# cbalint13/opencv-dlco

Hardware: AMD Instinct MI355X
Metric: pj-learn patch-pairs/sec (higher is better)
Workload: dtype f32; 1 GPU; pj-learn configs[1] Liberty-shaped, rank ~64: 500000 pair-rows x PR-dim 8192, batch 200+200 per GPU (global 200+200), mu=0.0025 gamma=0.5, fp32, rank 48 after 3893 steps; device= (gfx950:sramecc+:xnack-), burn_in_steps=300

## Files before the change

include/dlco.h:

```cpp
#ifndef DLCO_H
#define DLCO_H

#include <stddef.h>
#include <stdint.h>

#ifdef __cplusplus
extern "C" {
#endif

#define DLCO_OK            0
#define DLCO_ERR_INVALID  -2
#define DLCO_ERR_HIP      -3
#define DLCO_ERR_NODEVICE -4
#define DLCO_ERR_NOCONV   -5
#define DLCO_ERR_COMM     -6

typedef struct dlco_ctx dlco_ctx;

typedef struct dlco_cfg {
    int32_t  F;
    int32_t  N;
    int32_t  B;
    float    mu;
    float    gamma;
// ... 95 lines not shown
    int32_t split_k, k_dev, small_m_tiles, small_n_tiles, depth, reps;
    float   alpha, beta, b1, b2;
    const float *E1_host, *E2_host;
} dlco_gemm_probe_args;
int dlco_gemm_probe(dlco_ctx *ctx, const dlco_gemm_probe_args *args, float *C_host, float *C2_host, int32_t *depth_used,
                    double *us_per_launch);
int dlco_chol_probe(dlco_ctx *ctx, const float *M_host, int32_t n, int32_t ld, float rel_thresh, float *Linv_host,
                    int32_t *dead_host);
typedef struct dlco_ortho_probe_args {
    const float *Z_host, *Zprev_host, *Gp_host;
    int32_t m, panel_end, n_lock, unfused;
    float   alpha, b1, b2;
} dlco_ortho_probe_args;
int dlco_ortho_probe(dlco_ctx *ctx, const dlco_ortho_probe_args *args, float *Qo_host, float *Yb_host, float *T_host,
                     int64_t fused[2]);
int dlco_fused_counters(const dlco_ctx *ctx, int64_t out[2]);
int dlco_hinge_sum(dlco_ctx *ctx, const float *pos_host, int32_t n_pos,
                   const float *neg_host, int32_t n_neg, double *out);
int dlco_roc_stats(dlco_ctx *ctx, const float *dist_host, const uint8_t *labels_host, int32_t n,
                   float *fpr95, double *auc);

typedef struct dlco_log_entry {
    uint32_t t;
    int32_t  is_best;
    int32_t  saved;
    float    loss_val, regul, obj, obj_best;
    int32_t  rank, rank_best;
    int32_t  dim;
    double   auc, auc_best;
    float    fpr95, fpr95_best;
// ... 234 lines not shown
```

opencv-dlco_amd/__init__.py:

```python
import collections
import ctypes as C
import os
import subprocess

import numpy as np

_HERE = os.path.dirname(os.path.abspath(__file__))
LIB_PATH = os.path.join(_HERE, "libdlco.so")
HEADER_PATH = os.path.join(os.path.dirname(_HERE), "include", "dlco.h")

OK, ERR_INVALID, ERR_HIP, ERR_NODEVICE, ERR_NOCONV, ERR_COMM = 0, -2, -3, -4, -5, -6
BUF_DIST, BUF_GRAD, BUF_DFAVG, BUF_W, BUF_GATHER, BUF_DATA = 1, 2, 3, 4, 5, 6
ALLGATHER_FN = C.CFUNCTYPE(C.c_int, C.c_void_p, C.c_int32, C.c_size_t)
DETECT_THRESHOLD = 100 * 100 * 256 * 256


class DlcoError(RuntimeError):
    def __init__(self, code, msg):
        super().__init__("libdlco error %d: %s" % (code, msg))
        self.code = code


class Cfg(C.Structure):
    _fields_ = [
# ... 32 lines not shown
        ("A", GemmOperand), ("B", GemmOperand),
        ("B2_host", C.POINTER(C.c_float)),
        ("split_k", C.c_int32), ("k_dev", C.c_int32), ("small_m_tiles", C.c_int32), ("small_n_tiles", C.c_int32),
        ("depth", C.c_int32), ("reps", C.c_int32),
        ("alpha", C.c_float), ("beta", C.c_float), ("b1", C.c_float), ("b2", C.c_float),
        ("E1_host", C.POINTER(C.c_float)), ("E2_host", C.POINTER(C.c_float)),
    ]


class OrthoProbeArgs(C.Structure):
    _fields_ = [
        ("Z_host", C.POINTER(C.c_float)), ("Zprev_host", C.POINTER(C.c_float)), ("Gp_host", C.POINTER(C.c_float)),
        ("m", C.c_int32), ("panel_end", C.c_int32), ("n_lock", C.c_int32), ("unfused", C.c_int32),
        ("alpha", C.c_float), ("b1", C.c_float), ("b2", C.c_float),
    ]


def build(verbose=False):
    cmd = ["make", "-C", os.path.join(_HERE, "csrc"), "-j8"]
    if not verbose:
        cmd.insert(1, "-s")
    subprocess.check_call(cmd)


_lib = None
f32p, i32p, u8p, i64p = C.POINTER(C.c_float), C.POINTER(C.c_int32), C.POINTER(C.c_uint8), C.POINTER(C.c_int64)
f64p = C.POINTER(C.c_double)
_Line = collections.namedtuple("_Line", "dtype ptr dist dptr suffix")
_FLOAT, _BYTE = _Line(np.float32, f32p, np.float32, f32p, ""), _Line(np.uint8, u8p, np.int32, i32p, "_u8")

# ... 38 lines not shown
    L.dlco_get_W.argtypes = [vp, f32p, i32p]
    L.dlco_get_A.argtypes = [vp, f32p]
    L.dlco_get_dfavg.argtypes = [vp, f32p]
    L.dlco_set_state.argtypes = [vp, C.c_uint32, f32p, f32p, C.c_int32]
    L.dlco_validate.argtypes = [vp, f32p, f32p, i32p]
    L.dlco_stats.argtypes = [vp, f32p, C.c_int32, i32p, f32p, C.POINTER(C.c_double)]
    L.dlco_project_sqdist.argtypes = [vp, i32p, C.c_int32, f32p, C.c_int32, f32p]
    L.dlco_viol_counts.argtypes = [vp, f32p, f32p, C.c_int32, i32p, i32p]
    L.dlco_grad_rda.argtypes = [vp, i32p, i32p, i32p, i32p, C.c_int32, C.c_float, C.c_float, f32p, f32p]
    L.dlco_psd_project.argtypes = [vp, f32p, C.c_uint32, f32p, i32p, f32p]
    L.dlco_hinge_sum.argtypes = [vp, f32p, C.c_int32, f32p, C.c_int32, C.POINTER(C.c_double)]
    L.dlco_sym_product.argtypes = [vp, f32p, C.c_int32, f32p, C.c_int32, f32p]
    L.dlco_gemm_probe.argtypes = [vp, C.POINTER(GemmProbeArgs), f32p, f32p, i32p, C.POINTER(C.c_double)]
    L.dlco_chol_probe.argtypes = [vp, f32p, C.c_int32, C.c_int32, C.c_float, f32p, i32p]
    L.dlco_ortho_probe.argtypes = [vp, C.POINTER(OrthoProbeArgs), f32p, f32p, f32p, C.POINTER(C.c_int64)]
    L.dlco_fused_counters.argtypes = [vp, C.POINTER(C.c_int64)]
    L.dlco_roc_stats.argtypes = [vp, f32p, u8p, C.c_int32, f32p, C.POINTER(C.c_double)]
    L.dlco_log_step.argtypes = [vp, C.POINTER(LogEntry)]
    L.dlco_get_saved.argtypes = [vp, f32p, i32p, f32p]
    L.dlco_profile_enable.argtypes = [vp, C.c_int32]
    L.dlco_profile_read.argtypes = [vp, C.c_char_p, C.POINTER(C.c_int64), C.POINTER(C.c_double)]
    L.dlco_eig_stats.argtypes = [vp, C.POINTER(C.c_int64), C.POINTER(C.c_int64), C.POINTER(C.c_int64), i32p]
    L.dlco_counters.argtypes = [vp, C.POINTER(C.c_int64)]
    i64 = C.c_int64
    L.dlco_set_pairs_device.argtypes = [vp, vp, C.c_int32, i32p]
    L.dlco_desc_last_error.restype = C.c_char_p
    L.dlco_desc_last_error.argtypes = [vp]
    L.dlco_desc_create.argtypes = [C.POINTER(vp), C.c_float, C.c_int32, C.c_int32, C.c_int32]
    L.dlco_desc_destroy.argtypes = [vp]
    L.dlco_desc_destroy.restype = None
# ... 437 lines not shown
    def ortho_probe(self, Z, Gp, alpha, b1, b2=0.0, Zprev=None, panel_end=0, n_lock=0, unfused=False):
        z, gp = _f32(Z), _f32(Gp).ravel()
        zp = None if Zprev is None else _f32(Zprev)
        m, F = z.shape
        nt = F // 128
        assert F == self.F and F % 128 == 0 and gp.size == nt * (nt + 1) // 2 * 128 * 128 and (zp is None or zp.shape == z.shape)
        a = OrthoProbeArgs()
        a.Z_host, a.Zprev_host, a.Gp_host = _p(z, f32p), _p(zp, f32p), _p(gp, f32p)
        a.m, a.panel_end, a.n_lock, a.unfused = m, panel_end, n_lock, int(unfused)
        a.alpha, a.b1, a.b2 = alpha, b1, b2
        qo, yb, t = np.zeros((m, F), np.float32), np.zeros((m, F), np.float32), np.zeros((m, m), np.float32)
        fused = (C.c_int64 * 2)()
        self._ck(self.L.dlco_ortho_probe(self.h, C.byref(a), _p(qo, f32p), _p(yb, f32p), _p(t, f32p), fused))
        return dict(Qo=qo, Yb=yb, T=t, fused=fused[0], applied=fused[1])

    def hinge_sum(self, pos, neg):
        p, n = _f32(pos), _f32(neg)
        out = C.c_double()
        self._ck(self.L.dlco_hinge_sum(self.h, _p(p, f32p), p.size, _p(n, f32p), n.size, C.byref(out)))
        return out.value

    def roc_stats(self, dist, labels):
        d, l = _f32(dist), np.ascontiguousarray(labels, np.uint8).ravel()
        f, a = C.c_float(), C.c_double()
        self._ck(self.L.dlco_roc_stats(self.h, _p(d, f32p), _p(l, u8p), d.size, C.byref(f), C.byref(a)))
        return f.value, a.value

    def profile_enable(self, on=True):
        self._ck(self.L.dlco_profile_enable(self.h, int(on)))

# ... 739 lines not shown
```

opencv-dlco_amd/csrc/dlco_api.cpp:

```cpp
#include "../../include/dlco.h"

#include "dlco_internal.hpp"
#include "eig_tracker.hpp"
#include "pair_index.hpp"
#include "rccl_comm.hpp"
#include "host_comm.hpp"

#include <algorithm>
#include <cfloat>
#include <chrono>
#include <cmath>
#include <cstring>

using namespace dlco;

static thread_local std::string g_last_error;

namespace {
struct EnvSwitch { const char *name, *purpose; };
const EnvSwitch kEnvSwitches[] = {
    {"DLCO_SYRK_FP32", "gradient SYRK as the k-ordered fp32 MFMA chain (syrk_rda_kernel8) instead of split-bf16 planes"},
    {"DLCO_NO_PACKED", "full F x F dual average where the packed upper-tile form would apply"},
    {"DLCO_FORCE_SHARD", "column-sharded layout (cfg.shard) on a single rank: the multi-GPU path on one GPU"},
    {"DLCO_NO_RANK_UPDATE", "first filter term from a product with the dual average, not from the step's rank update"},
// ... 1272 lines not shown
        h2d(c, X.p, a->Z_host, rows * sizeof(float));
        if (a->Zprev_host) { Xprev.alloc(rows); h2d(c, Xprev.p, a->Zprev_host, rows * sizeof(float)); }
        h2d(c, Gp.p, a->Gp_host, syrk_packed_floats(F) * sizeof(float));
        EigTracker t(F, m, 8, c->cfg.eig_tol, c->cfg.eig_max_iter, c->stream);
        t.set_packed(true);
        t.set_fuse_gram(a->unfused == 0);
        t.ortho_probe(X.p, a->Zprev_host ? Xprev.p : nullptr, m, Gp.p, a->alpha, a->b1, a->b2, a->panel_end, a->n_lock, Qo.p, Yb.p, T.p);
        sync(c);
        d2h(c, Qo_host, Qo.p, rows * sizeof(float));
        d2h(c, Yb_host, Yb.p, rows * sizeof(float));
        d2h(c, T_host, T.p, (size_t)m * m * sizeof(float));
        if (fused) { fused[0] = t.stats().fused_gram_reductions; fused[1] = t.stats().fused_applications; }
    });
}

int dlco_fused_counters(const dlco_ctx *c, int64_t out[2])
{
    if (!c || !out) return DLCO_ERR_INVALID;
    out[0] = c->eig->stats().fused_gram_reductions;
    out[1] = c->eig->stats().fused_applications;
    return DLCO_OK;
}

int dlco_hinge_sum(dlco_ctx *c, const float *pos_host, int32_t n_pos, const float *neg_host, int32_t n_neg, double *out)
{
    if (!c || !out || n_pos < 0 || n_neg < 0) return DLCO_ERR_INVALID;
    return guarded(c, [&] {
        DLCO_HIP(hipSetDevice(c->cfg.device));
        *out = 0.0;
        if (n_pos == 0) return;
// ... 136 lines not shown
```

opencv-dlco_amd/csrc/dlco_internal.hpp:

```cpp
#pragma once

#include "../../include/dlco.h"
#include "match_batch.hpp"
#include "match_slices.hpp"
#include "select_rules.hpp"
#include "verify_batch.hpp"

#include <hip/hip_runtime.h>

#include <algorithm>
#include <climits>
#include <cstdint>
#include <cstdio>
#include <cstdlib>
#include <cstring>
#include <functional>
#include <mutex>
#include <utility>
#include <stdexcept>
#include <string>
#include <type_traits>
#include <vector>

namespace patch_rules { struct Frame; }
// ... 259 lines not shown
    const float *Y = nullptr, *Q = nullptr;
    long ld = 0;
    int m = 0, F = 0;
    float ay = 0.f, aq = 0.f, ac = 0.f;
    float *out = nullptr;
    int nw = 0;
    const float *wscale = nullptr;
    void *coeff_ws = nullptr;
    SplitPlanes out_planes;
};
bool rank_first_term(const RankTermBlock &b, const RankUpdate &ru, hipStream_t s);
size_t syrk_packed_floats(int F);
void syrk_pack_upper(const float *C, long ldc, int F, float *packed, hipStream_t s);
void syrk_unpack_upper(const float *packed, int F, float *C, long ldc, hipStream_t s);
bool skinny_product_sym(const SkinnyArgs &a, hipStream_t s);
bool reduce_gram_sym(const SkinnyArgs &a, hipStream_t s);
struct LinvApplyArgs {
    const float *Linv = nullptr;
    long ldl = 0;
    int n = 0, F = 0;
    const float *src = nullptr;
    float *dst = nullptr;
    long ld = 0;
    float *gram_slab = nullptr;
    int gram_chunk = 0;
    SplitPlanes planes;
};
bool linv_apply_slab(const LinvApplyArgs &a, hipStream_t s);
size_t gemm_slab_floats(int M, int N, int split_k);
inline int split_k_slices(long tiles, long target, long K, long kmin, long slab_cap)
// ... 160 lines not shown
```

opencv-dlco_amd/csrc/kernels_bf16x2.hip:

```cpp
#include "dlco_internal.hpp"
#include "split_bf16_dev.hpp"

#include <algorithm>

namespace dlco {

namespace {

constexpr int W8 = 8;
constexpr int T8 = 64 * W8;
constexpr int KS = 4;

__global__ __launch_bounds__(256) void split_x_kernel(const float *X, long ldx, int M, int MT, int K, bf16x8 *hi, bf16x8 *lo,
                                                      bf16x8 *lo2)
{
    const long t = (long)blockIdx.x * blockDim.x + threadIdx.x;
    const long total = (long)(K / 16) * MT * 64;
    if (t >= total) return;
    const int lane = (int)(t & 63);
    const long q = t >> 6;
    const int tile = (int)(q % MT);
    const int k16 = (int)(q / MT);
    const int row = tile * 32 + (lane & 31), k = k16 * 16 + 8 * (lane >> 5);
    bf16x8 h, l, l2;
// ... 223 lines not shown
            for (int r = 0; r < 16; r++) {
                const float sum = acc[a][r] + red[((nt * MT + a) * 16 + r) * 64 + lane];
                const int i = a * 32 + (r & 3) + 8 * (r >> 2) + 4 * lh;
                if (i < g.M) slab[(long)i * g.N + col] = sum;
            }
    }
}

__global__ __launch_bounds__(256) void reduce_split_kernel(const float *slab, int split, int M, int MT, int N, float *C, long ldc, float alpha,
                                                           const float *E1, float b1, const float *E2, float b2, bf16x8 *hi, bf16x8 *lo)
{
    const long total = (long)M * N, q = N >> 3;
    for (long e = (long)blockIdx.x * blockDim.x + threadIdx.x; e < (long)M * q; e += (long)gridDim.x * blockDim.x) {
        const int i = (int)(e / q), k8 = (int)(e % q), j = k8 * 8;
        const float *p = slab + (long)i * N + j;
        f32x4 s0 = *reinterpret_cast<const f32x4 *>(p), s1 = *reinterpret_cast<const f32x4 *>(p + 4);
        for (int z = 1; z < split; z++) {
            s0 += *reinterpret_cast<const f32x4 *>(p + (long)z * total);
            s1 += *reinterpret_cast<const f32x4 *>(p + (long)z * total + 4);
        }
        const long idx = (long)i * ldc + j;
        f32x4 o0 = alpha * s0, o1 = alpha * s1;
        if (E1) { o0 += b1 * *reinterpret_cast<const f32x4 *>(E1 + idx); o1 += b1 * *reinterpret_cast<const f32x4 *>(E1 + idx + 4); }
        if (E2) { o0 += b2 * *reinterpret_cast<const f32x4 *>(E2 + idx); o1 += b2 * *reinterpret_cast<const f32x4 *>(E2 + idx + 4); }
        *reinterpret_cast<f32x4 *>(C + idx) = o0;
        *reinterpret_cast<f32x4 *>(C + idx + 4) = o1;
        bf16x8 h, l, l2;
        split_frag<2>(o0, o1, h, l, l2);
        const long t = plane_entry_at(MT, i, k8);
        hi[t] = h;
        lo[t] = l;
    }
}

struct ReduceGramDev {
    const float *slab;
    int M, F;
    float *C;
    long ldc;
// ... 494 lines not shown
    ReduceGramDev r;
    r.slab = a.slab; r.M = M; r.F = F;
    r.C = a.C; r.ldc = a.ldc;
    r.alpha = a.alpha; r.E1 = a.E1; r.b1 = a.b1; r.E2 = a.E2; r.b2 = a.b2;
    r.tree = splitk_reduce_is_wide(a.slab, 4, M, F, a.C, a.ldc, a.E1, a.E2) ? 0 : 1;
    r.Y = a.gram_with; r.ldy = a.gram_ld;
    r.gram = a.gram_slab; r.chunk = a.gram_chunk;
    dispatch_mt<3>((M + 31) / 32, [&](auto MT) {
        if (a.gram_with) launch_reduce_gram<MT(), false>(r, s);
        else launch_reduce_gram<MT(), true>(r, s);
    });
    DLCO_HIP(hipGetLastError());
    return true;
}

bool skinny_product_sym(const SkinnyArgs &a, hipStream_t s)
{
    const int M = a.M, F = a.K;
    void *plane_hi = a.planes.hi, *plane_lo = a.planes.lo, *plane_lo2 = a.planes.lo2;
    const int mt = (M + 31) / 32;
    const int nt = F / 128;
    if (a.N != F || F % 128 != 0 || nt < 1 || nt > 64 || M < 1 || mt > 5 || (mt >= 4 && plane_lo2)) return false;
    if (a.ldx % 4 != 0 || (reinterpret_cast<uintptr_t>(a.X) & 15) != 0 || (reinterpret_cast<uintptr_t>(a.G) & 15) != 0) return false;
    if (a.emit_planes && plane_lo2) return false;
    if (!a.planes_ready) split_planes_bf16(a.X, a.ldx, M, F, plane_hi, plane_lo, plane_lo2, s);
    SymDev g;
    g.M = M; g.K = F;
    g.nt = nt; g.lb = 2;
    while ((1 << g.lb) < nt) g.lb++;
    g.xhi = static_cast<const bf16x8 *>(plane_hi); g.xlo = static_cast<const bf16x8 *>(plane_lo); g.xlo2 = static_cast<const bf16x8 *>(plane_lo2);
    g.G = a.G; g.slab = a.slab;
    if (plane_lo2) dispatch_mt<3>(mt, [&](auto MT) { launch_sym<MT(), 3>(g, s); });
    else dispatch_mt<5>(mt, [&](auto MT) { launch_sym<MT(), 2>(g, s); });
    DLCO_HIP(hipGetLastError());
    if (a.emit_planes && a.ldc % 4 == 0 && (reinterpret_cast<uintptr_t>(a.C) & 15) == 0) {
        const long work = (long)M * (F / 8);
        hipLaunchKernelGGL(reduce_split_kernel, dim3((unsigned)std::min<long>((work + 255) / 256, 4096)), dim3(256), 0, s, a.slab, 4, M, mt, F, a.C, a.ldc,
                           a.alpha, a.E1, a.b1, a.E2, a.b2, static_cast<bf16x8 *>(plane_hi), static_cast<bf16x8 *>(plane_lo));
        DLCO_HIP(hipGetLastError());
    } else if (reduce_gram_sym(a, s)) {
        if (a.gram_done) *a.gram_done = true;
    } else {
        splitk_reduce_f32(a.slab, 4, M, F, a.C, a.ldc, a.alpha, 0.f, a.E1, a.b1, a.E2, a.b2, s);
    }
    return true;
}

}
```

opencv-dlco_amd/csrc/kernels_eig.hip:

```cpp
#include "dlco_internal.hpp"

#include <type_traits>

namespace dlco {

namespace {

typedef float f32x4 __attribute__((ext_vector_type(4)));

__device__ __forceinline__ float wsum(float v)
{
#pragma unroll
    for (int o = 32; o > 0; o >>= 1) v += __shfl_xor(v, o, 64);
    return v;
}

__global__ __launch_bounds__(256) void residual_kernel(const float *X, const float *Y, long ld, const float *theta,
                                                       int m, int F, float *res)
{
    __shared__ float part[4];
    const int i = blockIdx.x;
    if (i >= m) return;
    const float th = theta[i];
    float s = 0.f;
    if ((F & 3) == 0 && (ld & 3) == 0) {
        const f32x4 *y4 = reinterpret_cast<const f32x4 *>(Y + (long)i * ld), *x4 = reinterpret_cast<const f32x4 *>(X + (long)i * ld);
        for (int f = threadIdx.x; f < F / 4; f += blockDim.x) {
            const f32x4 d = y4[f] - th * x4[f];
            s += d[0] * d[0] + d[1] * d[1] + d[2] * d[2] + d[3] * d[3];
        }
    } else {
        for (int f = threadIdx.x; f < F; f += blockDim.x) {
            const float d = Y[(long)i * ld + f] - th * X[(long)i * ld + f];
            s += d * d;
        }
    }
    s = wsum(s);
    if ((threadIdx.x & 63) == 0) part[threadIdx.x >> 6] = s;
    __syncthreads();
    if (threadIdx.x == 0) res[i] = sqrtf(part[0] + part[1] + part[2] + part[3]);
}

__global__ __launch_bounds__(256) void row_normalize_kernel(float *X, long ld, int m, int F, float min_norm)
{
    __shared__ float part[4];
    __shared__ float inv;
    const int i = blockIdx.x;
    if (i >= m) return;
    float s = 0.f;
    const bool vec = (F & 3) == 0 && (ld & 3) == 0;
    f32x4 *x4 = reinterpret_cast<f32x4 *>(X + (long)i * ld);
// ... 285 lines not shown
                             hipStream_t s)
{
    chol_inverse_dispatch<true>(M, ldm, n, rel_thresh, Linv, ldl, dead, trace, s);
}

__global__ __launch_bounds__(256) void residual_publish_kernel(const float *X, const float *Y, long ld, const float *theta, int m, int F,
                                                               float *res, unsigned *ticket, const float *src, float *dst_host, int n,
                                                               unsigned *flag_host, unsigned seq, const int *extra_dev, int *extra_host,
                                                               ResidualEmit em)
{
    __shared__ float part[4];
    __shared__ int last;
    __shared__ int cnt[4];
    const int i = blockIdx.x;
    const float th = theta[i];
    float s = 0.f;
    if (em.W && (F & 3) == 0 && (ld & 3) == 0 && (em.ldw & 3) == 0) {
        int c = 0;
        for (int k = threadIdx.x; k < m; k += blockDim.x) c += theta[k] > em.mu ? 1 : 0;
        c = (int)wsum((float)c);
        if ((threadIdx.x & 63) == 0) cnt[threadIdx.x >> 6] = c;
        __syncthreads();
        const int nw = cnt[0] + cnt[1] + cnt[2] + cnt[3];
        const bool mine = i < nw || em.guards;
        const float sc = i < nw ? sqrtf(em.cscale * (th - em.mu)) : 1.0f;
        f32x4 *w4 = reinterpret_cast<f32x4 *>(em.W + (long)(i < nw ? nw - 1 - i : i) * em.ldw);
        if (em.wscale && threadIdx.x == 0) em.wscale[i] = sc;
        const f32x4 *y4 = reinterpret_cast<const f32x4 *>(Y + (long)i * ld), *x4 = reinterpret_cast<const f32x4 *>(X + (long)i * ld);
        for (int f = threadIdx.x; f < F / 4; f += blockDim.x) {
            const f32x4 x = x4[f];
            const f32x4 d = y4[f] - th * x;
            s += d[0] * d[0] + d[1] * d[1] + d[2] * d[2] + d[3] * d[3];
            if (mine) { f32x4 v = x; v[0] *= sc; v[1] *= sc; v[2] *= sc; v[3] *= sc; w4[f] = v; }
        }
    } else if ((F & 3) == 0 && (ld & 3) == 0) {
        const f32x4 *y4 = reinterpret_cast<const f32x4 *>(Y + (long)i * ld), *x4 = reinterpret_cast<const f32x4 *>(X + (long)i * ld);
        for (int f = threadIdx.x; f < F / 4; f += blockDim.x) {
            const f32x4 d = y4[f] - th * x4[f];
            s += d[0] * d[0] + d[1] * d[1] + d[2] * d[2] + d[3] * d[3];
        }
    } else {
        for (int f = threadIdx.x; f < F; f += blockDim.x) {
            const float d = Y[(long)i * ld + f] - th * X[(long)i * ld + f];
            s += d * d;
        }
    }
    s = wsum(s);
    if ((threadIdx.x & 63) == 0) part[threadIdx.x >> 6] = s;
    __syncthreads();
    if (threadIdx.x == 0) {
        __hip_atomic_store(res + i, sqrtf(part[0] + part[1] + part[2] + part[3]), __ATOMIC_RELAXED, __HIP_MEMORY_SCOPE_AGENT);
        const unsigned t = __hip_atomic_fetch_add(ticket, 1u, __ATOMIC_ACQ_REL, __HIP_MEMORY_SCOPE_AGENT);
        last = t == gridDim.x - 1 ? 1 : 0;
        if (last) __hip_atomic_store(ticket, 0u, __ATOMIC_RELAXED, __HIP_MEMORY_SCOPE_AGENT);
    }
    __syncthreads();
    if (!last) return;
    __builtin_amdgcn_fence(__ATOMIC_ACQUIRE, "agent");
    for (int k = threadIdx.x; k < n; k += 256) dst_host[k] = __hip_atomic_load(src + k, __ATOMIC_RELAXED, __HIP_MEMORY_SCOPE_AGENT);
    if (extra_dev && threadIdx.x == 0) *extra_host = __hip_atomic_load(extra_dev, __ATOMIC_RELAXED, __HIP_MEMORY_SCOPE_AGENT);
// ... 39 lines not shown
```

opencv-dlco_amd/csrc/kernels_step.hip:

```cpp
#include "dlco_internal.hpp"

#include <algorithm>

namespace dlco {

namespace {

__device__ __forceinline__ double wave_sum_d(double v)
{
#pragma unroll
    for (int o = 32; o > 0; o >>= 1) v += __shfl_xor(v, o, 64);
    return v;
}

__global__ void sqdist_kernel(const float *proj, int split, int r, int n, long ld, float *dist)
{
    const int j = blockIdx.x * blockDim.x + threadIdx.x;
    if (j >= n) return;
    const long plane = (long)r * ld;
    float d = 0.f;
    int q = 0;
    if (split == 1) {
        for (; q + 8 <= r; q += 8) {
            float v[8];
#pragma unroll
            for (int u = 0; u < 8; u++) v[u] = proj[(long)(q + u) * ld + j];
#pragma unroll
            for (int u = 0; u < 8; u++) d += v[u] * v[u];
        }
    }
    for (; q < r; q++) {
        float p = 0.f;
        for (int z = 0; z < split; z++) p += proj[z * plane + (long)q * ld + j];
        d += p * p;
    }
    dist[j] = d;
}

__global__ __launch_bounds__(512) void sqdist_split_kernel(const float *proj, int split, int r, int n, long ld, float *dist, int r_all,
                                                           float *reduced)
{
    __shared__ float p[96][64];
    const int jl = threadIdx.x & 63, qg = threadIdx.x >> 6;
    const int j = blockIdx.x * 64 + jl;
// ... 14 lines not shown
                    for (int u = 0; u < 8; u++) acc += v[u];
                }
                for (; z < split; z++) acc += src[z * plane];
            }
            p[q][jl] = acc;
            if (reduced && j < n) reduced[(long)(q0 + q) * ld + j] = acc;
        }
        __syncthreads();
        if (qg == 0)
            for (int q = 0; q < min(qn, r - q0); q++) d += p[q][jl] * p[q][jl];
        __syncthreads();
    }
    if (qg == 0 && j < n) dist[j] = d;
}

__device__ __forceinline__ void viol_body(float *sh, const float *pd, const float *nd, int B, int32_t *rho, int32_t *kappa)
{
    float *spd = sh, *snd = sh + B;
    for (int i = threadIdx.x; i < B; i += blockDim.x) { spd[i] = pd[i] + 1.0f; snd[i] = nd[i]; }
    __syncthreads();
    for (int i = threadIdx.x; i < B; i += blockDim.x) {
        const float thr = spd[i];
        int c = 0;
        for (int j = 0; j < B; j++) c += (thr > snd[j]) ? 1 : 0;
        rho[i] = c;
        const float me = snd[i];
        int k = 0;
        for (int j = 0; j < B; j++) k += (spd[j] > me) ? 1 : 0;
        kappa[i] = k;
    }
}
__global__ void viol_kernel(const float *pd, const float *nd, int B, int32_t *rho, int32_t *kappa)
{
    extern __shared__ float sh[];
    viol_body(sh, pd, nd, B, rho, kappa);
}

__device__ __forceinline__ void active_rows_body(const int32_t *pos_rows, const int32_t *neg_rows, const int32_t *rho,
                                                 const int32_t *kappa, int B, int lo, int hi, int32_t *ids, float *w, int *k_active,
                                                 int32_t *slots = nullptr)
{
    __shared__ int wave_cnt[16];
    __shared__ int base;
    const int tid = threadIdx.x, lane = tid & 63, wave = tid >> 6, nw = blockDim.x >> 6;
    const int n_own = max(0, min(hi, B) - lo), total = 2 * n_own;
    if (tid == 0) base = 0;
    __syncthreads();
    for (int c0 = 0; c0 < total; c0 += blockDim.x) {
        const int e = c0 + tid;
        int id = 0;
        float wt = 0.f;
        bool keep = false;
        if (e < total) {
            if (e < n_own) { const int i = lo + e; keep = rho[i] != 0; id = pos_rows[i]; wt = (float)rho[i]; }
            else { const int j = lo + e - n_own; keep = kappa[j] != 0; id = neg_rows[j]; wt = -(float)kappa[j]; }
        }
        const unsigned long long m = __ballot(keep);
        if (lane == 0) wave_cnt[wave] = __popcll(m);
        __syncthreads();
        int off = base;
        for (int v = 0; v < wave; v++) off += wave_cnt[v];
        if (keep) {
            const int pos = off + __popcll(m & ((1ull << lane) - 1ull));
            ids[pos] = id;
            w[pos] = wt;
            if (slots) slots[pos] = e;
        }
        __syncthreads();
        if (tid == 0) { int s = 0; for (int v = 0; v < nw; v++) s += wave_cnt[v]; base += s; }
        __syncthreads();
    }
    const int k = base;
    if (tid == 0) *k_active = k;
    for (int z = k + tid; z < ((2 * B + 31) & ~31); z += blockDim.x) { ids[z] = 0; w[z] = 0.f; }
}
__global__ void active_rows_kernel(const int32_t *pos_rows, const int32_t *neg_rows, const int32_t *rho,
                                   const int32_t *kappa, int B, int lo, int hi, int32_t *ids, float *w, int *k_active)
{
    active_rows_body(pos_rows, neg_rows, rho, kappa, B, lo, hi, ids, w, k_active);
}
__global__ void viol_active_kernel(const float *pd, const float *nd, int B, int32_t *rho, int32_t *kappa, const int32_t *pos_rows,
                                   const int32_t *neg_rows, int lo, int hi, int32_t *ids, float *w, int *k_active, int32_t *slots)
{
    extern __shared__ float sh[];
    viol_body(sh, pd, nd, B, rho, kappa);
    __threadfence_block();
    __syncthreads();
    active_rows_body(pos_rows, neg_rows, rho, kappa, B, lo, hi, ids, w, k_active, slots);
}

__global__ __launch_bounds__(256) void hinge_rows_kernel(const float *pos, int n_pos, const float *neg, int n_neg,
                                                         float *row_sums, long ld_in, long ld_out)
{
    __shared__ float sn[2048];
    pos += blockIdx.y * ld_in;
    neg += blockIdx.y * ld_in;
    row_sums += blockIdx.y * ld_out;
    const int i = blockIdx.x * blockDim.x + threadIdx.x;
    const float base = (i < n_pos) ? pos[i] + 1.0f : 0.f;
    float tsum = 0.f;
    for (int j0 = 0; j0 < n_neg; j0 += 2048) {
        const int cnt = min(2048, n_neg - j0);
        __syncthreads();
// ... 143 lines not shown

void viol_counts(const float *pd, const float *nd, int B, int32_t *rho, int32_t *kappa, hipStream_t s)
{
    if (B <= 0) return;
    DLCO_CHECK(B <= 8192, -2, "viol_counts: batch too large for one workgroup's LDS");
    hipLaunchKernelGGL(viol_kernel, dim3(1), dim3(256), 2 * B * sizeof(float), s, pd, nd, B, rho, kappa);
    DLCO_HIP(hipGetLastError());
}

void viol_counts_active_rows(const float *pd, const float *nd, int B, int32_t *rho, int32_t *kappa, const int32_t *pos_rows,
                             const int32_t *neg_rows, int slot_lo, int slot_hi, int32_t *ids, float *w, int *k_active, int32_t *slots,
                             hipStream_t s)
{
    if (B <= 0) return;
    DLCO_CHECK(B <= 8192, -2, "viol_counts: batch too large for one workgroup's LDS");
    hipLaunchKernelGGL(viol_active_kernel, dim3(1), dim3(256), 2 * B * sizeof(float), s, pd, nd, B, rho, kappa, pos_rows, neg_rows, slot_lo,
                       slot_hi, ids, w, k_active, slots);
    DLCO_HIP(hipGetLastError());
}

void build_active_rows(const int32_t *pos_rows, const int32_t *neg_rows, const int32_t *rho, const int32_t *kappa,
                       int B, int slot_lo, int slot_hi, int32_t *ids, float *w, int *k_active, hipStream_t s)
{
    hipLaunchKernelGGL(active_rows_kernel, dim3(1), dim3(256), 0, s, pos_rows, neg_rows, rho, kappa, B, slot_lo, slot_hi,
                       ids, w, k_active);
    DLCO_HIP(hipGetLastError());
}

void hinge_rows(const float *pos, int n_pos, const float *neg, int n_neg, float *row_sums, hipStream_t s)
{
    if (n_pos <= 0) return;
    hipLaunchKernelGGL(hinge_rows_kernel, dim3((n_pos + 255) / 256), dim3(256), 0, s, pos, n_pos, neg, n_neg, row_sums, 0L, 0L);
// ... 94 lines not shown
```

Baseline: 752,100 pair-rows/s.

## Batch loads in split reduction, residual, sqdist and violation kernels; add step probes

Several small per-step kernels are restructured so that more global loads are in flight before use. The split-K reduce issues all slab and epilogue loads up front. Residual rows use a shared helper, and theta counting is unrolled. sqdist loads 64 rows per pass and keeps the order of its adds. The violation/active-rows kernel keeps rho/kappa in LDS and prefetches candidate row ids before the counting phase. A step-probe API is added for testing these kernels. The cost is larger LDS use and more registers, which may need an opt-in for dynamic LDS and could lower occupancy.

```diff
diff --git a/include/dlco.h b/include/dlco.h
--- a/include/dlco.h
+++ b/include/dlco.h
@@ -133,6 +133,27 @@
 } dlco_ortho_probe_args;
 int dlco_ortho_probe(dlco_ctx *ctx, const dlco_ortho_probe_args *args, float *Qo_host, float *Yb_host, float *T_host,
                      int64_t fused[2]);
+enum { DLCO_STEP_PROBE_REDUCE_SPLIT = 0, DLCO_STEP_PROBE_RESIDUAL = 1, DLCO_STEP_PROBE_SQDIST = 2, DLCO_STEP_PROBE_VIOL_ACTIVE = 3 };
+typedef struct dlco_step_probe_args {
+    int32_t kernel, m, n, split;
+    const float *slab, *E1, *E2;
+    float        alpha, b1, b2;
+    float       *C;
+    uint16_t    *hi, *lo;
+    const float *X, *Y, *theta;
+    int32_t      publish, emit, guards;
+    uint32_t     seq;
+    float        mu, cscale;
+    float       *res, *W, *wscale, *published;
+    uint32_t    *flag;
+    const float *proj;
+    float       *dist;
+    const float *pd, *nd;
+    const int32_t *pos_rows, *neg_rows;
+    int32_t     *rho, *kappa, *ids, *slots, *k_active;
+    float       *w;
+} dlco_step_probe_args;
+int dlco_step_probe(dlco_ctx *ctx, const dlco_step_probe_args *args);
 int dlco_fused_counters(const dlco_ctx *ctx, int64_t out[2]);
 int dlco_hinge_sum(dlco_ctx *ctx, const float *pos_host, int32_t n_pos,
                    const float *neg_host, int32_t n_neg, double *out);
diff --git a/opencv-dlco_amd/__init__.py b/opencv-dlco_amd/__init__.py
--- a/opencv-dlco_amd/__init__.py
+++ b/opencv-dlco_amd/__init__.py
@@ -70,6 +70,29 @@
         ("m", C.c_int32), ("panel_end", C.c_int32), ("n_lock", C.c_int32), ("unfused", C.c_int32),
         ("alpha", C.c_float), ("b1", C.c_float), ("b2", C.c_float),
     ]
+
+
+class StepProbeArgs(C.Structure):
+    _fields_ = [
+        ("kernel", C.c_int32), ("m", C.c_int32), ("n", C.c_int32), ("split", C.c_int32),
+        ("slab", C.POINTER(C.c_float)), ("E1", C.POINTER(C.c_float)), ("E2", C.POINTER(C.c_float)),
+        ("alpha", C.c_float), ("b1", C.c_float), ("b2", C.c_float),
+        ("C", C.POINTER(C.c_float)), ("hi", C.POINTER(C.c_uint16)), ("lo", C.POINTER(C.c_uint16)),
+        ("X", C.POINTER(C.c_float)), ("Y", C.POINTER(C.c_float)), ("theta", C.POINTER(C.c_float)),
+        ("publish", C.c_int32), ("emit", C.c_int32), ("guards", C.c_int32), ("seq", C.c_uint32),
+        ("mu", C.c_float), ("cscale", C.c_float),
+        ("res", C.POINTER(C.c_float)), ("W", C.POINTER(C.c_float)), ("wscale", C.POINTER(C.c_float)),
+        ("published", C.POINTER(C.c_float)), ("flag", C.POINTER(C.c_uint32)),
+        ("proj", C.POINTER(C.c_float)), ("dist", C.POINTER(C.c_float)),
+        ("pd", C.POINTER(C.c_float)), ("nd", C.POINTER(C.c_float)),
+        ("pos_rows", C.POINTER(C.c_int32)), ("neg_rows", C.POINTER(C.c_int32)),
+        ("rho", C.POINTER(C.c_int32)), ("kappa", C.POINTER(C.c_int32)), ("ids", C.POINTER(C.c_int32)),
+        ("slots", C.POINTER(C.c_int32)), ("k_active", C.POINTER(C.c_int32)),
+        ("w", C.POINTER(C.c_float)),
+    ]
+
+
+STEP_PROBE_REDUCE_SPLIT, STEP_PROBE_RESIDUAL, STEP_PROBE_SQDIST, STEP_PROBE_VIOL_ACTIVE = 0, 1, 2, 3
 
 
 def build(verbose=False):
@@ -138,6 +161,7 @@
     L.dlco_gemm_probe.argtypes = [vp, C.POINTER(GemmProbeArgs), f32p, f32p, i32p, C.POINTER(C.c_double)]
     L.dlco_chol_probe.argtypes = [vp, f32p, C.c_int32, C.c_int32, C.c_float, f32p, i32p]
     L.dlco_ortho_probe.argtypes = [vp, C.POINTER(OrthoProbeArgs), f32p, f32p, f32p, C.POINTER(C.c_int64)]
+    L.dlco_step_probe.argtypes = [vp, C.POINTER(StepProbeArgs)]
     L.dlco_fused_counters.argtypes = [vp, C.POINTER(C.c_int64)]
     L.dlco_roc_stats.argtypes = [vp, f32p, u8p, C.c_int32, f32p, C.POINTER(C.c_double)]
     L.dlco_log_step.argtypes = [vp, C.POINTER(LogEntry)]
@@ -605,6 +629,51 @@
         self._ck(self.L.dlco_ortho_probe(self.h, C.byref(a), _p(qo, f32p), _p(yb, f32p), _p(t, f32p), fused))
         return dict(Qo=qo, Yb=yb, T=t, fused=fused[0], applied=fused[1])
 
+    def _step_probe(self, kernel, m, n, keep, **fields):
+        a = StepProbeArgs()
+        a.kernel, a.m, a.n = kernel, m, n
+        types = dict(StepProbeArgs._fields_)
+        for name, v in fields.items():
+            setattr(a, name, _p(v, types[name]) if isinstance(v, np.ndarray) or v is None else v)
+        self._ck(self.L.dlco_step_probe(self.h, C.byref(a)))
+        return keep
+
+    def reduce_split_probe(self, slab, alpha=1.0, E1=None, b1=0.0, E2=None, b2=0.0):
+        s = _f32(slab)
+        split, m, n = s.shape
+        e1, e2 = (None if e is None else _f32(e) for e in (E1, E2))
+        assert all(e is None or e.shape == (m, n) for e in (e1, e2))
+        out = dict(C=np.zeros((m, n), np.float32), hi=np.zeros((m + 31) // 32 * 32 * n, np.uint16), lo=np.zeros((m + 31) // 32 * 32 * n, np.uint16))
+        return self._step_probe(STEP_PROBE_REDUCE_SPLIT, m, n, out, split=split, slab=s, E1=e1, E2=e2, alpha=alpha, b1=b1, b2=b2, **out)
+
+    def residual_probe(self, X, Y, theta, publish=True, emit=False, guards=False, mu=0.0, cscale=1.0, seq=1, fill=-7.0):
+        x, y, th = _f32(X), _f32(Y), _f32(theta)
+        m, n = x.shape
+        assert y.shape == x.shape and th.shape == (m,)
+        out = dict(res=np.full(m, fill, np.float32))
+        if publish:
+            out.update(published=np.full(m, fill, np.float32), flag=np.zeros(1, np.uint32))
+        if emit:
+            out.update(W=np.full((m, n), fill, np.float32), wscale=np.full(m, fill, np.float32))
+        return self._step_probe(STEP_PROBE_RESIDUAL, m, n, out, X=x, Y=y, theta=th, publish=int(publish), emit=int(emit), guards=int(guards), seq=seq,
+                                mu=mu, cscale=cscale, **out)
+
+    def sqdist_probe(self, proj):
+        p = _f32(proj)
+        r, n = p.shape
+        dist = np.zeros(n, np.float32)
+        self._step_probe(STEP_PROBE_SQDIST, r, n, None, proj=p, dist=dist)
+        return dist
+
+    def viol_active_probe(self, pd, nd, pos_rows, neg_rows, fill=-7):
+        p, q, pr, nr = _f32(pd), _f32(nd), _i32(pos_rows), _i32(neg_rows)
+        B = p.size
+        assert q.size == B and pr.size == B and nr.size == B
+        kcap = (2 * B + 31) // 32 * 32
+        out = dict(rho=np.full(B, fill, np.int32), kappa=np.full(B, fill, np.int32), ids=np.full(kcap, fill, np.int32), w=np.full(kcap, fill, np.float32),
+                   slots=np.full(2 * B, fill, np.int32), k_active=np.full(1, fill, np.int32))
+        return self._step_probe(STEP_PROBE_VIOL_ACTIVE, 1, B, out, pd=p, nd=q, pos_rows=pr, neg_rows=nr, **out)
+
     def hinge_sum(self, pos, neg):
         p, n = _f32(pos), _f32(neg)
         out = C.c_double()
diff --git a/opencv-dlco_amd/csrc/dlco_api.cpp b/opencv-dlco_amd/csrc/dlco_api.cpp
--- a/opencv-dlco_amd/csrc/dlco_api.cpp
+++ b/opencv-dlco_amd/csrc/dlco_api.cpp
@@ -1310,6 +1310,107 @@
     });
 }
 
+int dlco_step_probe(dlco_ctx *c, const dlco_step_probe_args *a)
+{
+    if (!c || !a || a->m < 1 || a->n < 1) return DLCO_ERR_INVALID;
+    return guarded(c, [&] {
+        DLCO_HIP(hipSetDevice(c->cfg.device));
+        const int m = a->m, n = a->n;
+        const size_t mn = (size_t)m * n;
+        auto up = [&](auto &buf, const auto *host, size_t count) {
+            buf.alloc(count);
+            h2d(c, buf.p, host, count * sizeof(*host));
+        };
+        auto down = [&](auto *host, const auto &buf, size_t count) { d2h(c, host, buf.p, count * sizeof(*host)); };
+        switch (a->kernel) {
+        case DLCO_STEP_PROBE_REDUCE_SPLIT: {
+            DLCO_CHECK(a->slab && a->C && a->hi && a->lo && a->split >= 1 && n % 16 == 0 && m <= 160, DLCO_ERR_INVALID, "dlco_step_probe: reduce_split arguments");
+            const size_t plane = (size_t)((m + 31) / 32) * 32 * n;
+            DevBuf<float> slab, E1, E2, C;
+            DevBuf<uint16_t> hi, lo;
+            up(slab, a->slab, (size_t)a->split * mn);
+            if (a->E1) up(E1, a->E1, mn);
+            if (a->E2) up(E2, a->E2, mn);
+            up(C, a->C, mn); up(hi, a->hi, plane); up(lo, a->lo, plane);
+            reduce_split_planes(slab.p, a->split, m, n, C.p, n, a->alpha, a->E1 ? E1.p : nullptr, a->b1, a->E2 ? E2.p : nullptr, a->b2, hi.p, lo.p,
+                                c->stream);
+            sync(c);
+            down(a->C, C, mn); down(a->hi, hi, plane); down(a->lo, lo, plane);
+            break;
+        }
+        case DLCO_STEP_PROBE_RESIDUAL: {
+            DLCO_CHECK(a->X && a->Y && a->theta && a->res && m <= 4096, DLCO_ERR_INVALID, "dlco_step_probe: residual arguments");
+            DLCO_CHECK(!a->emit || (a->publish && a->W && a->wscale), DLCO_ERR_INVALID, "dlco_step_probe: emission needs the publishing launch, W and wscale");
+            DLCO_CHECK(!a->publish || (a->published && a->flag), DLCO_ERR_INVALID, "dlco_step_probe: published / flag missing");
+            DevBuf<float> X, Y, theta, res, W, wscale;
+            up(X, a->X, mn); up(Y, a->Y, mn); up(theta, a->theta, (size_t)m); up(res, a->res, (size_t)m);
+            if (!a->publish) {
+                residual_norms(X.p, Y.p, n, theta.p, m, n, res.p, c->stream);
+                sync(c);
+                down(a->res, res, (size_t)m);
+                break;
+            }
+            DevBuf<unsigned> ticket;
+            ticket.alloc(1);
+            ticket.zero(c->stream);
+            struct Pin {
+                float *p = nullptr;
+                ~Pin() { if (p) (void)hipHostFree(p); }
+            } pin;
+            DLCO_HIP(hipHostMalloc((void **)&pin.p, ((size_t)m + 1) * sizeof(float), hipHostMallocCoherent));
+            std::memcpy(pin.p, a->published, (size_t)m * sizeof(float));
+            unsigned *flag = reinterpret_cast<unsigned *>(pin.p + m);
+            *flag = *a->flag;
+            ResidualPublish rp;
+            rp.X = X.p; rp.Y = Y.p; rp.ld = n; rp.theta = theta.p; rp.m = m; rp.F = n; rp.res = res.p;
+            rp.ticket = ticket.p;
+            rp.src = res.p; rp.dst_host = pin.p; rp.n = m;
+            rp.flag_host = flag; rp.seq = a->seq;
+            if (a->emit) {
+                up(W, a->W, mn); up(wscale, a->wscale, (size_t)m);
+                rp.emit.W = W.p; rp.emit.ldw = n; rp.emit.mu = a->mu; rp.emit.cscale = a->cscale;
+                rp.emit.wscale = wscale.p; rp.emit.guards = a->guards != 0;
+            }
+            const bool emitted = residual_norms_publish(rp, c->stream);
+            sync(c);
+            DLCO_CHECK(!a->emit || emitted, DLCO_ERR_INVALID, "dlco_step_probe: n must be a multiple of 4 for the launch to emit W");
+            down(a->res, res, (size_t)m);
+            std::memcpy(a->published, pin.p, (size_t)m * sizeof(float));
+            *a->flag = __atomic_load_n(flag, __ATOMIC_ACQUIRE);
+            if (a->emit) { down(a->W, W, mn); down(a->wscale, wscale, (size_t)m); }
+            break;
+        }
+        case DLCO_STEP_PROBE_SQDIST: {
+            DLCO_CHECK(a->proj && a->dist, DLCO_ERR_INVALID, "dlco_step_probe: sqdist arguments");
+            DevBuf<float> proj, dist;
+            up(proj, a->proj, mn); up(dist, a->dist, (size_t)n);
+            sqdist_from_proj(proj.p, 1, m, n, n, dist.p, c->stream);
+            sync(c);
+            down(a->dist, dist, (size_t)n);
+            break;
+        }
+        case DLCO_STEP_PROBE_VIOL_ACTIVE: {
+            DLCO_CHECK(a->pd && a->nd && a->pos_rows && a->neg_rows && a->rho && a->kappa && a->ids && a->w && a->slots && a->k_active && n <= 8192,
+                       DLCO_ERR_INVALID, "dlco_step_probe: viol_active arguments");
+            const size_t B = (size_t)n, kcap = (2 * B + 31) & ~(size_t)31;
+            DevBuf<float> pd, nd, w;
+            DevBuf<int32_t> pos, neg, rho, kappa, ids, slots;
+            DevBuf<int> k;
+            up(pd, a->pd, B); up(nd, a->nd, B); up(pos, a->pos_rows, B); up(neg, a->neg_rows, B);
+            up(rho, a->rho, B); up(kappa, a->kappa, B); up(ids, a->ids, kcap); up(w, a->w, kcap); up(slots, a->slots, 2 * B);
+            up(k, a->k_active, (size_t)1);
+            viol_counts_active_rows(pd.p, nd.p, n, rho.p, kappa.p, pos.p, neg.p, 0, n, ids.p, w.p, k.p, slots.p, c->stream);
+            sync(c);
+            down(a->rho, rho, B); down(a->kappa, kappa, B); down(a->ids, ids, kcap); down(a->w, w, kcap); down(a->slots, slots, 2 * B);
+            down(a->k_active, k, (size_t)1);
+            break;
+        }
+        default:
+            DLCO_CHECK(false, DLCO_ERR_INVALID, "dlco_step_probe: unknown kernel");
+        }
+    });
+}
+
 int dlco_fused_counters(const dlco_ctx *c, int64_t out[2])
 {
     if (!c || !out) return DLCO_ERR_INVALID;
diff --git a/opencv-dlco_amd/csrc/dlco_internal.hpp b/opencv-dlco_amd/csrc/dlco_internal.hpp
--- a/opencv-dlco_amd/csrc/dlco_internal.hpp
+++ b/opencv-dlco_amd/csrc/dlco_internal.hpp
@@ -297,6 +297,8 @@
 void syrk_pack_upper(const float *C, long ldc, int F, float *packed, hipStream_t s);
 void syrk_unpack_upper(const float *packed, int F, float *C, long ldc, hipStream_t s);
 bool skinny_product_sym(const SkinnyArgs &a, hipStream_t s);
+void reduce_split_planes(const float *slab, int split, int M, int F, float *C, long ldc, float alpha, const float *E1, float b1,
+                         const float *E2, float b2, void *hi, void *lo, hipStream_t s);
 bool reduce_gram_sym(const SkinnyArgs &a, hipStream_t s);
 struct LinvApplyArgs {
     const float *Linv = nullptr;
diff --git a/opencv-dlco_amd/csrc/kernels_bf16x2.hip b/opencv-dlco_amd/csrc/kernels_bf16x2.hip
--- a/opencv-dlco_amd/csrc/kernels_bf16x2.hip
+++ b/opencv-dlco_amd/csrc/kernels_bf16x2.hip
@@ -261,15 +261,34 @@
     for (long e = (long)blockIdx.x * blockDim.x + threadIdx.x; e < (long)M * q; e += (long)gridDim.x * blockDim.x) {
         const int i = (int)(e / q), k8 = (int)(e % q), j = k8 * 8;
         const float *p = slab + (long)i * N + j;
-        f32x4 s0 = *reinterpret_cast<const f32x4 *>(p), s1 = *reinterpret_cast<const f32x4 *>(p + 4);
-        for (int z = 1; z < split; z++) {
-            s0 += *reinterpret_cast<const f32x4 *>(p + (long)z * total);
-            s1 += *reinterpret_cast<const f32x4 *>(p + (long)z * total + 4);
-        }
         const long idx = (long)i * ldc + j;
+        auto ld4 = [](const float *q) { return *reinterpret_cast<const f32x4 *>(q); };
+        const f32x4 zero = {0.f, 0.f, 0.f, 0.f};
+        const f32x4 e10 = E1 ? ld4(E1 + idx) : zero, e11 = E1 ? ld4(E1 + idx + 4) : zero;
+        const f32x4 e20 = E2 ? ld4(E2 + idx) : zero, e21 = E2 ? ld4(E2 + idx + 4) : zero;
+        f32x4 s0, s1;
+        if (split == 4) {
+            f32x4 v0[4], v1[4];
+#pragma unroll
+            for (int z = 0; z < 4; z++) { v0[z] = ld4(p + (long)z * total); v1[z] = ld4(p + (long)z * total + 4); }
+            s0 = v0[0]; s1 = v1[0];
+#pragma unroll
+            for (int z = 1; z < 4; z++) { s0 += v0[z]; s1 += v1[z]; }
+        } else {
+            s0 = ld4(p); s1 = ld4(p + 4);
+            int z = 1;
+            for (; z + 4 <= split; z += 4) {
+                f32x4 v0[4], v1[4];
+#pragma unroll
+                for (int u = 0; u < 4; u++) { v0[u] = ld4(p + (long)(z + u) * total); v1[u] = ld4(p + (long)(z + u) * total + 4); }
+#pragma unroll
+                for (int u = 0; u < 4; u++) { s0 += v0[u]; s1 += v1[u]; }
+            }
+            for (; z < split; z++) { s0 += ld4(p + (long)z * total); s1 += ld4(p + (long)z * total + 4); }
+        }
         f32x4 o0 = alpha * s0, o1 = alpha * s1;
-        if (E1) { o0 += b1 * *reinterpret_cast<const f32x4 *>(E1 + idx); o1 += b1 * *reinterpret_cast<const f32x4 *>(E1 + idx + 4); }
-        if (E2) { o0 += b2 * *reinterpret_cast<const f32x4 *>(E2 + idx); o1 += b2 * *reinterpret_cast<const f32x4 *>(E2 + idx + 4); }
+        if (E1) { o0 += b1 * e10; o1 += b1 * e11; }
+        if (E2) { o0 += b2 * e20; o1 += b2 * e21; }
         *reinterpret_cast<f32x4 *>(C + idx) = o0;
         *reinterpret_cast<f32x4 *>(C + idx + 4) = o1;
         bf16x8 h, l, l2;
@@ -794,6 +813,16 @@
     return true;
 }
 
+void reduce_split_planes(const float *slab, int split, int M, int F, float *C, long ldc, float alpha, const float *E1, float b1,
+                         const float *E2, float b2, void *hi, void *lo, hipStream_t s)
+{
+    DLCO_CHECK(M >= 1 && split >= 1 && F >= 8 && F % 8 == 0 && ldc % 4 == 0, -2, "reduce_split_planes: shape");
+    const long work = (long)M * (F / 8);
+    hipLaunchKernelGGL(reduce_split_kernel, dim3((unsigned)std::min<long>((work + 255) / 256, 4096)), dim3(256), 0, s, slab, split, M, (M + 31) / 32, F, C,
+                       ldc, alpha, E1, b1, E2, b2, static_cast<bf16x8 *>(hi), static_cast<bf16x8 *>(lo));
+    DLCO_HIP(hipGetLastError());
+}
+
 bool skinny_product_sym(const SkinnyArgs &a, hipStream_t s)
 {
     const int M = a.M, F = a.K;
@@ -814,10 +843,7 @@
     else dispatch_mt<5>(mt, [&](auto MT) { launch_sym<MT(), 2>(g, s); });
     DLCO_HIP(hipGetLastError());
     if (a.emit_planes && a.ldc % 4 == 0 && (reinterpret_cast<uintptr_t>(a.C) & 15) == 0) {
-        const long work = (long)M * (F / 8);
-        hipLaunchKernelGGL(reduce_split_kernel, dim3((unsigned)std::min<long>((work + 255) / 256, 4096)), dim3(256), 0, s, a.slab, 4, M, mt, F, a.C, a.ldc,
-                           a.alpha, a.E1, a.b1, a.E2, a.b2, static_cast<bf16x8 *>(plane_hi), static_cast<bf16x8 *>(plane_lo));
-        DLCO_HIP(hipGetLastError());
+        reduce_split_planes(a.slab, 4, M, F, a.C, a.ldc, a.alpha, a.E1, a.b1, a.E2, a.b2, plane_hi, plane_lo, s);
     } else if (reduce_gram_sym(a, s)) {
         if (a.gram_done) *a.gram_done = true;
     } else {
diff --git a/opencv-dlco_amd/csrc/kernels_eig.hip b/opencv-dlco_amd/csrc/kernels_eig.hip
--- a/opencv-dlco_amd/csrc/kernels_eig.hip
+++ b/opencv-dlco_amd/csrc/kernels_eig.hip
@@ -13,6 +13,45 @@
 #pragma unroll
     for (int o = 32; o > 0; o >>= 1) v += __shfl_xor(v, o, 64);
     return v;
+}
+
+__device__ __forceinline__ float residual_term(float s, float x, float y, float th)
+{
+    const float d = __fmaf_rn(-th, x, y);
+    return __fmaf_rn(d, d, s);
+}
+__device__ __forceinline__ float residual_term(float s, const f32x4 &x, const f32x4 &y, float th)
+{
+#pragma clang fp contract(off)
+    float q[4];
+#pragma unroll
+    for (int k = 0; k < 4; k++) { const float d = __fmaf_rn(-th, x[k], y[k]); q[k] = d * d; }
+    return s + (((q[0] + q[1]) + q[2]) + q[3]);
+}
+__device__ __forceinline__ float scaled(float x, float sc) { return x * sc; }
+__device__ __forceinline__ f32x4 scaled(f32x4 v, float sc) { v[0] *= sc; v[1] *= sc; v[2] *= sc; v[3] *= sc; return v; }
+
+template <bool EMIT, typename V>
+__device__ __forceinline__ float residual_row(const V *x, const V *y, int n, float th, bool mine = false, float sc = 1.0f, V *w = nullptr)
+{
+    constexpr int G = 8, T = 256;
+    float s = 0.f;
+    for (int f0 = threadIdx.x; f0 < n; f0 += G * T) {
+        V xv[G], yv[G];
+#pragma unroll
+        for (int t = 0; t < G; t++) {
+            const int f = f0 + t * T < n ? f0 + t * T : f0;
+            xv[t] = x[f];
+            yv[t] = y[f];
+        }
+#pragma unroll
+        for (int t = 0; t < G; t++) {
+            const bool have = f0 + t * T < n;
+            s = have ? residual_term(s, xv[t], yv[t], th) : s;
+            if (EMIT && mine && have) w[f0 + t * T] = scaled(xv[t], sc);
+        }
+    }
+    return s;
 }
 
 __global__ __launch_bounds__(256) void residual_kernel(const float *X, const float *Y, long ld, const float *theta,
@@ -22,19 +61,11 @@
     const int i = blockIdx.x;
     if (i >= m) return;
     const float th = theta[i];
-    float s = 0.f;
-    if ((F & 3) == 0 && (ld & 3) == 0) {
-        const f32x4 *y4 = reinterpret_cast<const f32x4 *>(Y + (long)i * ld), *x4 = reinterpret_cast<const f32x4 *>(X + (long)i * ld);
-        for (int f = threadIdx.x; f < F / 4; f += blockDim.x) {
-            const f32x4 d = y4[f] - th * x4[f];
-            s += d[0] * d[0] + d[1] * d[1] + d[2] * d[2] + d[3] * d[3];
-        }
-    } else {
-        for (int f = threadIdx.x; f < F; f += blockDim.x) {
-            const float d = Y[(long)i * ld + f] - th * X[(long)i * ld + f];
-            s += d * d;
-        }
-    }
+    float s;
+    if ((F & 3) == 0 && (ld & 3) == 0)
+        s = residual_row<false>(reinterpret_cast<const f32x4 *>(X + (long)i * ld), reinterpret_cast<const f32x4 *>(Y + (long)i * ld), F / 4, th);
+    else
+        s = residual_row<false>(X + (long)i * ld, Y + (long)i * ld, F, th);
     s = wsum(s);
     if ((threadIdx.x & 63) == 0) part[threadIdx.x >> 6] = s;
     __syncthreads();
@@ -350,10 +381,16 @@
     __shared__ int cnt[4];
     const int i = blockIdx.x;
     const float th = theta[i];
-    float s = 0.f;
+    float s;
     if (em.W && (F & 3) == 0 && (ld & 3) == 0 && (em.ldw & 3) == 0) {
         int c = 0;
-        for (int k = threadIdx.x; k < m; k += blockDim.x) c += theta[k] > em.mu ? 1 : 0;
+        for (int k0 = threadIdx.x; k0 < m; k0 += 4 * 256) {
+            float t[4];
+#pragma unroll
+            for (int u = 0; u < 4; u++) t[u] = theta[k0 + u * 256 < m ? k0 + u * 256 : k0];
+#pragma unroll
+            for (int u = 0; u < 4; u++) c += k0 + u * 256 < m && t[u] > em.mu ? 1 : 0;
+        }
         c = (int)wsum((float)c);
         if ((threadIdx.x & 63) == 0) cnt[threadIdx.x >> 6] = c;
         __syncthreads();
@@ -362,24 +399,11 @@
         const float sc = i < nw ? sqrtf(em.cscale * (th - em.mu)) : 1.0f;
         f32x4 *w4 = reinterpret_cast<f32x4 *>(em.W + (long)(i < nw ? nw - 1 - i : i) * em.ldw);
         if (em.wscale && threadIdx.x == 0) em.wscale[i] = sc;
-        const f32x4 *y4 = reinterpret_cast<const f32x4 *>(Y + (long)i * ld), *x4 = reinterpret_cast<const f32x4 *>(X + (long)i * ld);
-        for (int f = threadIdx.x; f < F / 4; f += blockDim.x) {
-            const f32x4 x = x4[f];
-            const f32x4 d = y4[f] - th * x;
-            s += d[0] * d[0] + d[1] * d[1] + d[2] * d[2] + d[3] * d[3];
-            if (mine) { f32x4 v = x; v[0] *= sc; v[1] *= sc; v[2] *= sc; v[3] *= sc; w4[f] = v; }
-        }
+        s = residual_row<true>(reinterpret_cast<const f32x4 *>(X + (long)i * ld), reinterpret_cast<const f32x4 *>(Y + (long)i * ld), F / 4, th, mine, sc, w4);
     } else if ((F & 3) == 0 && (ld & 3) == 0) {
-        const f32x4 *y4 = reinterpret_cast<const f32x4 *>(Y + (long)i * ld), *x4 = reinterpret_cast<const f32x4 *>(X + (long)i * ld);
-        for (int f = threadIdx.x; f < F / 4; f += blockDim.x) {
-            const f32x4 d = y4[f] - th * x4[f];
-            s += d[0] * d[0] + d[1] * d[1] + d[2] * d[2] + d[3] * d[3];
-        }
+        s = residual_row<false>(reinterpret_cast<const f32x4 *>(X + (long)i * ld), reinterpret_cast<const f32x4 *>(Y + (long)i * ld), F / 4, th);
     } else {
-        for (int f = threadIdx.x; f < F; f += blockDim.x) {
-            const float d = Y[(long)i * ld + f] - th * X[(long)i * ld + f];
-            s += d * d;
-        }
+        s = residual_row<false>(X + (long)i * ld, Y + (long)i * ld, F, th);
     }
     s = wsum(s);
     if ((threadIdx.x & 63) == 0) part[threadIdx.x >> 6] = s;
diff --git a/opencv-dlco_amd/csrc/kernels_step.hip b/opencv-dlco_amd/csrc/kernels_step.hip
--- a/opencv-dlco_amd/csrc/kernels_step.hip
+++ b/opencv-dlco_amd/csrc/kernels_step.hip
@@ -11,6 +11,13 @@
 #pragma unroll
     for (int o = 32; o > 0; o >>= 1) v += __shfl_xor(v, o, 64);
     return v;
+}
+
+__device__ __forceinline__ float add_square_rounded(float d, float v)
+{
+#pragma clang fp contract(off)
+    const float q = v * v;
+    return d + q;
 }
 
 __global__ void sqdist_kernel(const float *proj, int split, int r, int n, long ld, float *dist)
@@ -21,13 +28,31 @@
     float d = 0.f;
     int q = 0;
     if (split == 1) {
-        for (; q + 8 <= r; q += 8) {
-            float v[8];
-#pragma unroll
-            for (int u = 0; u < 8; u++) v[u] = proj[(long)(q + u) * ld + j];
-#pragma unroll
-            for (int u = 0; u < 8; u++) d += v[u] * v[u];
-        }
+        float tail[7];
+#pragma unroll
+        for (int u = 0; u < 7; u++) tail[u] = 0.f;
+        const int qt = r & ~7;
+        if (r & 7) {
+#pragma unroll
+            for (int u = 0; u < 7; u++) tail[u] = proj[(long)(qt + u < r ? qt + u : qt) * ld + j];
+        }
+        for (; q + 8 <= r; q += 64) {
+            float v[64];
+#pragma unroll
+            for (int b = 0; b < 8; b++)
+                if (q + 8 * b + 8 <= r) {
+#pragma unroll
+                    for (int u = 0; u < 8; u++) v[8 * b + u] = proj[(long)(q + 8 * b + u) * ld + j];
+                } else {
+#pragma unroll
+                    for (int u = 0; u < 8; u++) v[8 * b + u] = 0.f;
+                }
+#pragma unroll
+            for (int u = 0; u < 64; u++) d = q + (u | 7) < r ? add_square_rounded(d, v[u]) : d;
+        }
+#pragma unroll
+        for (int u = 0; u < 7; u++) d = qt + u < r ? __fmaf_rn(tail[u], tail[u], d) : d;
+        q = r;
     }
     for (; q < r; q++) {
         float p = 0.f;
@@ -72,7 +97,8 @@
     if (qg == 0 && j < n) dist[j] = d;
 }
 
-__device__ __forceinline__ void viol_body(float *sh, const float *pd, const float *nd, int B, int32_t *rho, int32_t *kappa)
+__device__ __forceinline__ void viol_body(float *sh, const float *pd, const float *nd, int B, int32_t *rho, int32_t *kappa,
+                                          int32_t *srho = nullptr, int32_t *skappa = nullptr)
 {
     float *spd = sh, *snd = sh + B;
     for (int i = threadIdx.x; i < B; i += blockDim.x) { spd[i] = pd[i] + 1.0f; snd[i] = nd[i]; }
@@ -82,10 +108,12 @@
         int c = 0;
         for (int j = 0; j < B; j++) c += (thr > snd[j]) ? 1 : 0;
         rho[i] = c;
+        if (srho) srho[i] = c;
         const float me = snd[i];
         int k = 0;
         for (int j = 0; j < B; j++) k += (spd[j] > me) ? 1 : 0;
         kappa[i] = k;
+        if (skappa) skappa[i] = k;
     }
 }
 __global__ void viol_kernel(const float *pd, const float *nd, int B, int32_t *rho, int32_t *kappa)
@@ -94,9 +122,16 @@
     viol_body(sh, pd, nd, B, rho, kappa);
 }
 
+__device__ __forceinline__ int32_t candidate_row(const int32_t *pos_rows, const int32_t *neg_rows, int lo, int n_own, int e)
+{
+    if (e >= 2 * n_own) return 0;
+    return e < n_own ? pos_rows[lo + e] : neg_rows[lo + e - n_own];
+}
+constexpr int ACT_PRE = 2;
+
 __device__ __forceinline__ void active_rows_body(const int32_t *pos_rows, const int32_t *neg_rows, const int32_t *rho,
                                                  const int32_t *kappa, int B, int lo, int hi, int32_t *ids, float *w, int *k_active,
-                                                 int32_t *slots = nullptr)
+                                                 int32_t *slots = nullptr, const int32_t *pre = nullptr)
 {
     __shared__ int wave_cnt[16];
     __shared__ int base;
@@ -104,14 +139,20 @@
     const int n_own = max(0, min(hi, B) - lo), total = 2 * n_own;
     if (tid == 0) base = 0;
     __syncthreads();
-    for (int c0 = 0; c0 < total; c0 += blockDim.x) {
+    for (int c0 = 0, chunk = 0; c0 < total; c0 += blockDim.x, chunk++) {
         const int e = c0 + tid;
         int id = 0;
         float wt = 0.f;
         bool keep = false;
+        if (pre && chunk < ACT_PRE) {
+#pragma unroll
+            for (int u = 0; u < ACT_PRE; u++) id = chunk == u ? pre[u] : id;
+        } else {
+            id = candidate_row(pos_rows, neg_rows, lo, n_own, e);
+        }
         if (e < total) {
-            if (e < n_own) { const int i = lo + e; keep = rho[i] != 0; id = pos_rows[i]; wt = (float)rho[i]; }
-            else { const int j = lo + e - n_own; keep = kappa[j] != 0; id = neg_rows[j]; wt = -(float)kappa[j]; }
+            if (e < n_own) { const int i = lo + e; keep = rho[i] != 0; wt = (float)rho[i]; }
+            else { const int j = lo + e - n_own; keep = kappa[j] != 0; wt = -(float)kappa[j]; }
         }
         const unsigned long long m = __ballot(keep);
         if (lane == 0) wave_cnt[wave] = __popcll(m);
@@ -141,10 +182,14 @@
                                    const int32_t *neg_rows, int lo, int hi, int32_t *ids, float *w, int *k_active, int32_t *slots)
 {
     extern __shared__ float sh[];
-    viol_body(sh, pd, nd, B, rho, kappa);
-    __threadfence_block();
+    int32_t pre[ACT_PRE];
+    const int n_own = max(0, min(hi, B) - lo);
+#pragma unroll
+    for (int u = 0; u < ACT_PRE; u++) pre[u] = candidate_row(pos_rows, neg_rows, lo, n_own, u * (int)blockDim.x + (int)threadIdx.x);
+    int32_t *srho = reinterpret_cast<int32_t *>(sh + 2 * B), *skappa = srho + B;
+    viol_body(sh, pd, nd, B, rho, kappa, srho, skappa);
     __syncthreads();
-    active_rows_body(pos_rows, neg_rows, rho, kappa, B, lo, hi, ids, w, k_active, slots);
+    active_rows_body(pos_rows, neg_rows, srho, skappa, B, lo, hi, ids, w, k_active, slots, pre);
 }
 
 __global__ __launch_bounds__(256) void hinge_rows_kernel(const float *pos, int n_pos, const float *neg, int n_neg,
@@ -318,8 +363,10 @@
 {
     if (B <= 0) return;
     DLCO_CHECK(B <= 8192, -2, "viol_counts: batch too large for one workgroup's LDS");
-    hipLaunchKernelGGL(viol_active_kernel, dim3(1), dim3(256), 2 * B * sizeof(float), s, pd, nd, B, rho, kappa, pos_rows, neg_rows, slot_lo,
-                       slot_hi, ids, w, k_active, slots);
+    const size_t lds = (size_t)4 * B * sizeof(float);
+    if (lds > 65536) ensure_dynamic_lds(reinterpret_cast<const void *>(viol_active_kernel), 4 * 8192 * (int)sizeof(float));
+    hipLaunchKernelGGL(viol_active_kernel, dim3(1), dim3(256), lds, s, pd, nd, B, rho, kappa, pos_rows, neg_rows, slot_lo, slot_hi, ids, w,
+                       k_active, slots);
     DLCO_HIP(hipGetLastError());
 }
 
```

Result: no change. 755,900 pair-rows/s (median of 4 runs) (+0.5%).
